# ru-wang/slam-plus-plus

Hardware: AMD Instinct MI355X
Metric: Λ-solve block-nnz/sec + batch GN iters/sec, Venice BA, 1→8 MI355X (higher is better)
Workload: dtype f64; 1 GPU; venice871-shaped synthetic BA (871 cams, 530304 points, 2838740 observations, LM-damped); nnzb=3369915, n=1596138, mode=schur+dense, n_reduced=5226, schur_pairs=12875640, parallelism=single GPU

## Files before the change

slam_plus_plus_amd/csrc/spp_api.cpp:

```cpp

#include "spp_internal.h"
#include <string.h>
#include <new>

using namespace spp;

namespace spp {

void phases_reset(spp_ctx *ctx)
{
	if(!(ctx->flags & SPP_FLAG_PROFILE))
		return;
	if(!ctx->timer.created) {
		for(int i = 0; i < 2 * SPP_N_PHASES; ++ i)
			SPP_HIP_CHECK(hipEventCreate(&ctx->timer.ev[i]));
		ctx->timer.created = true;
	}
	for(int i = 0; i < SPP_N_PHASES; ++ i) {
		ctx->timer.used[i] = false;
		ctx->phase_ms[i] = 0;
	}
	ctx->dom_used = 0;
	ctx->dom_flops = 0;
}
// ... 23 lines not shown
			continue;
		float ms = 0;
		if(hipEventElapsedTime(&ms, ctx->timer.ev[2 * i], ctx->timer.ev[2 * i + 1]) == hipSuccess)
			ctx->phase_ms[i] = ms;
	}
}

void dom_begin(spp_ctx *ctx)
{
	if(!(ctx->flags & SPP_FLAG_PROFILE))
		return;
	if(ctx->dom_used + 2 > ctx->dom_events.size()) {
		size_t old = ctx->dom_events.size();
		ctx->dom_events.resize(old + 64);
		for(size_t i = old; i < ctx->dom_events.size(); ++ i)
			SPP_HIP_CHECK(hipEventCreate(&ctx->dom_events[i]));
	}
	SPP_HIP_CHECK(hipEventRecord(ctx->dom_events[ctx->dom_used], ctx->stream));
}

void dom_end(spp_ctx *ctx, double flops)
{
	if(!(ctx->flags & SPP_FLAG_PROFILE))
		return;
	SPP_HIP_CHECK(hipEventRecord(ctx->dom_events[ctx->dom_used + 1], ctx->stream));
	ctx->dom_used += 2;
	ctx->dom_flops += flops;
}

}

#define SPP_TRY(ctx) try {
#define SPP_CATCH(ctx) } catch(const spp::Error &e) { if(ctx) (ctx)->last_error = e.what(); return e.code; } \
	catch(const std::bad_alloc &) { if(ctx) (ctx)->last_error = "host allocation failed"; return SPP_E_NOMEM; } \
	catch(const std::exception &e) { if(ctx) (ctx)->last_error = e.what(); return SPP_E_HIP; }

extern "C" {

const char *spp_version(void)
{
	return "slam_plus_plus_amd 0.1 (gfx950, fp64)";
}

spp_ctx *spp_create(int device, int flags)
{
	int count = 0;
	if(hipGetDeviceCount(&count) != hipSuccess || count <= 0 || device < 0 || device >= count)
		return nullptr;
	if(hipSetDevice(device) != hipSuccess)
		return nullptr;
	spp_ctx *ctx = new(std::nothrow) spp_ctx;
	if(!ctx)
		return nullptr;
	ctx->device = device;
	ctx->flags = flags;
	if(hipStreamCreateWithFlags(&ctx->stream, hipStreamNonBlocking) != hipSuccess) {
		delete ctx;
		return nullptr;
	}
	ctx->own_stream = true;
	return ctx;
}

int spp_free_memory(spp_ctx *ctx)
{
	if(!ctx)
		return SPP_E_BADARG;
	SPP_TRY(ctx)
	(void)hipSetDevice(ctx->device);
	(void)hipStreamSynchronize(ctx->stream);
	ctx->schur.release_all();
	sparse_release(ctx);
	assemble_release(ctx);
	ctx->dense.tinv.release();
	ctx->dense.tinv_all.release();
	ctx->dense.xtmp.release();
	ctx->dense.la_cnt.release();
	ctx->dense.la_trace.release();
	ctx->geom_partial.release();
	ctx->dense.flags.release();
	ctx->dense.trsv_pay.release();
	ctx->dense.trsv_m.release();
	ctx->dense.tail_pub.release();
	ctx->dense.tail_order.release();
	ctx->dense.tail_order_tr = ctx->dense.tail_order_tc = 0;
	ctx->dense.tail_dinv.release();
	ctx->dense.tail_epoch = 0;
	ctx->dense.epoch = 0;
	ctx->dense.sync.release();
	ctx->dense.fuse_cnt.release();
	ctx->dense.fuse_expect.clear();
	ctx->dense.sync_epoch = 0;
	ctx->d_vals.release();
	ctx->d_rhs.release();
	ctx->mode = -1;
	return SPP_OK;
	SPP_CATCH(ctx)
}

void spp_destroy(spp_ctx *ctx)
{
	if(!ctx)
		return;
	if(ctx->plan_trash.joinable())
		ctx->plan_trash.join();
	spp_free_memory(ctx);
	ctx->dense.info.release();
	if(ctx->dense.aux) {
		dense_aux_park(ctx->device, ctx->dense.aux);
		(void)hipEventDestroy(ctx->dense.ev[0]);
		(void)hipEventDestroy(ctx->dense.ev[1]);
	}
	if(ctx->dense.chain) {
		(void)hipStreamDestroy(ctx->dense.chain);
		if(ctx->dense.ev_chain)
			(void)hipEventDestroy(ctx->dense.ev_chain);
	}
	if(ctx->dense.h_chain_err)
		(void)hipHostFree(ctx->dense.h_chain_err);
	if(ctx->h_staging)
		(void)hipHostFree(ctx->h_staging);
	if(ctx->timer.created)
		for(int i = 0; i < 2 * SPP_N_PHASES; ++ i)
			(void)hipEventDestroy(ctx->timer.ev[i]);
	for(size_t i = 0; i < ctx->dom_events.size(); ++ i)
		(void)hipEventDestroy(ctx->dom_events[i]);
	if(ctx->own_stream && ctx->stream)
		(void)hipStreamDestroy(ctx->stream);
	delete ctx;
}

int spp_last_error(const spp_ctx *ctx, char *buf, size_t buf_size)
{
	if(!ctx || !buf || !buf_size)
		return SPP_E_BADARG;
	strncpy(buf, ctx->last_error.c_str(), buf_size - 1);
	buf[buf_size - 1] = 0;
	return SPP_OK;
}

double *spp_host_staging(spp_ctx *ctx, int64_t n_doubles)
{
	if(!ctx || n_doubles < 0)
		return nullptr;
	if((size_t)n_doubles <= ctx->h_staging_cap && ctx->h_staging)
		return ctx->h_staging;
	(void)hipSetDevice(ctx->device);
	(void)hipStreamSynchronize(ctx->stream);
	if(ctx->h_staging) {
		(void)hipHostFree(ctx->h_staging);
		ctx->h_staging = nullptr;
		ctx->h_staging_cap = 0;
	}
	const size_t want = (size_t)(n_doubles > 0 ? n_doubles : 1);
	if(hipHostMalloc((void**)&ctx->h_staging, want * sizeof(double), hipHostMallocDefault) != hipSuccess) {
		(void)hipGetLastError();
		ctx->h_staging = nullptr;
		ctx->last_error = "hipHostMalloc of the staging buffer failed";
		return nullptr;
	}
	ctx->h_staging_cap = want;
	return ctx->h_staging;
}

int spp_set_stream(spp_ctx *ctx, void *hip_stream)
{
// ... 774 lines not shown
```

slam_plus_plus_amd/csrc/spp_dense.hip:

```cpp

#include "spp_internal.h"
#include "spp_tiles.h"
#include "spp_dense_dev.h"
#include <stdio.h>
#include <stdlib.h>
#include <string.h>
#include <algorithm>
#include <vector>
#include <mutex>

namespace spp {


constexpr int BK = 16;
constexpr int LDS_STRIDE = 18;

template <int BM, int BN, int WM, int WN, int MODE, int DEPTH, int BKT, int SC1 = 0>
__device__ __forceinline__ void gemm_tn_tile(const int64_t m0, const int64_t n0, int64_t M, int64_t N, int K,
	const double *__restrict__ A, int64_t lda, const double *B, int64_t ldb, double *C, int64_t ldc, double *gemm_lds)
{
	constexpr int NWM = BM / WM, NWN = BN / WN, NT = NWM * NWN * 64;
	constexpr int TA = WM / 16, TB = WN / 16;
	constexpr int PPC = BKT / 2, LSTR = BKT + 2;
	constexpr int PA = (BM * PPC) / NT, PB = (BN * PPC) / NT;
// ... 1176 lines not shown
	SPP_HIP_CHECK(hipEventRecord(dw.ev[1], sb));
	SPP_HIP_CHECK(hipEventRecord(dw.ev_chain, sc));
	SPP_HIP_CHECK(hipStreamWaitEvent(s, dw.ev[1], 0));
	SPP_HIP_CHECK(hipStreamWaitEvent(s, dw.ev_chain, 0));
	SPP_HIP_CHECK(hipGetLastError());
	if(tracing) {
		std::vector<long long> h((size_t)12 * nsteps + 16);
		SPP_HIP_CHECK(hipMemcpyAsync(h.data(), dw.la_trace.p, h.size() * sizeof(long long), hipMemcpyDeviceToHost, s));
		SPP_HIP_CHECK(hipStreamSynchronize(s));
		fprintf(stderr, "[spp] lookahead factorization, %d steps: potrf start / duration / gap to the next start (us)\n", a.nsteps);
		for(int k = 0; k < a.nsteps; ++ k)
			fprintf(stderr, "  k %2d  start %8.1f  potrf %5.1f  publish %4.1f | b1 seen +%4.1f  done +%4.1f | c1 seen +%4.1f  done +%4.1f | step %5.1f\n", k,
				(h[8 * k] - h[0]) * 0.01, (h[8 * k + 2] - h[8 * k]) * 0.01, (h[8 * k + 1] - h[8 * k + 2]) * 0.01,
				(h[8 * k + 3] - h[8 * k + 1]) * 0.01, (h[8 * k + 4] - h[8 * k + 1]) * 0.01, (h[8 * k + 5] - h[8 * k + 1]) * 0.01,
				(h[8 * k + 6] - h[8 * k + 1]) * 0.01, k + 1 < a.nsteps ? (h[8 * (k + 1)] - h[8 * k]) * 0.01 : 0.0);
		fprintf(stderr, "[spp] per step: panel (rest) done / bulk launch: first tile starts, priority tiles done, last tile done, busy workgroup-us (all relative to potrf(0) start)\n");
		for(int k = 0; k < a.nsteps; ++ k) {
			const long long *b = h.data() + 8 * nsteps + 8 + 4 * k;
			fprintf(stderr, "  k %2d  panel done %8.1f | bulk start %8.1f  pri done %8.1f  end %8.1f  busy %9.1f\n", k, h[8 * k + 7] ? (h[8 * k + 7] - h[0]) * 0.01 : 0.0,
				b[1] ? (b[0] - h[0]) * 0.01 : 0.0, b[3] ? (b[3] - h[0]) * 0.01 : 0.0, b[1] ? (b[1] - h[0]) * 0.01 : 0.0, b[2] * 0.01);
		}
	}
}

void dense_factor_steps(spp_ctx *ctx, double *d_A, int64_t ld, int64_t n, int64_t rows, int64_t ncols,
	int64_t nsteps, bool has_rhs)
{
	ensure_dense_work(ctx, nsteps);
	ctx->dense.tail_rows_last = 0;
	hipStreamCaptureStatus cs = hipStreamCaptureStatusNone;
	const bool capturing = hipStreamIsCapturing(ctx->stream, &cs) != hipSuccess || cs != hipStreamCaptureStatusNone;
	if(!capturing && la_usable(ctx, nsteps)) {
		dense_factor_lookahead(ctx, d_A, ld, n, rows, ncols, nsteps, has_rhs);
		ctx->dense.tinv_half = 0;
		return;
	}
	ctx->dense.tinv_half = nsteps;
	const bool flags = !capturing && nsteps >= 4 && flag_schedule_usable(ctx);
	dense_factor_steps_enqueue(ctx, d_A, ld, n, rows, ncols, nsteps, has_rhs, flags, !capturing);
}

static void flag_signal(hipStream_t st, int *flag, int value)
{
	hipLaunchKernelGGL(flag_signal_kernel, dim3(1), dim3(64), 0, st, flag, value);
}

static FlagWait make_flag_wait(spp_ctx *ctx, const int *flag, int value, double timeout_ms = 500.0)
{
	return FlagWait{flag, value, ctx->dense.info.p + 2, (long long)(timeout_ms * 1e5)};
}

static void flag_wait(spp_ctx *ctx, hipStream_t st, const int *flag, int value, double timeout_ms)
{
	hipLaunchKernelGGL(flag_wait_kernel, dim3(1), dim3(64), 0, st, make_flag_wait(ctx, flag, value, timeout_ms));
}

static bool flag_schedule_selftest(spp_ctx *ctx)
{
	DenseWork &dw = ctx->dense;
	hipStream_t st[2] = {ctx->stream, dw.aux};
	dw.sync.reserve(16);
	SPP_HIP_CHECK(hipMemsetAsync(dw.sync.p, 0, 16 * sizeof(int), ctx->stream));
	SPP_HIP_CHECK(hipStreamSynchronize(ctx->stream));
	for(int p = 0; p < 2; ++ p) {
		flag_wait(ctx, st[p], dw.sync.p + p, 1, 20.0);
		flag_signal(st[1 - p], dw.sync.p + p, 1);
	}
	for(int i = 0; i < 2; ++ i)
		SPP_HIP_CHECK(hipStreamSynchronize(st[i]));
	int h_abort = 0;
	SPP_HIP_CHECK(hipMemcpy(&h_abort, dw.info.p + 2, sizeof(int), hipMemcpyDeviceToHost));
	if(h_abort) {
		SPP_HIP_CHECK(hipMemset(dw.info.p + 2, 0, sizeof(int)));
		return false;
	}
	return true;
}

static bool flag_schedule_usable(spp_ctx *ctx)
{
	static int sched = -1;
	if(sched < 0) {
		const char *e = getenv("SPP_DENSE_SCHED");
		sched = e ? atoi(e) : 1;
	}
	if(!sched)
		return false;
	DenseWork &dw = ctx->dense;
	if(dw.sync_state == 0 || dw.sync_stream != ctx->stream) {
		hipStreamCaptureStatus cs = hipStreamCaptureStatusNone;
		if(hipStreamIsCapturing(ctx->stream, &cs) != hipSuccess || cs != hipStreamCaptureStatusNone)
			return false;
		dw.sync_state = flag_schedule_selftest(ctx) ? 1 : -1;
		dw.sync_stream = ctx->stream;
	}
	return dw.sync_state == 1;
}

static int dense_tail_rows()
{
	static int v = -1;
	if(v < 0) {
		const char *e = getenv("SPP_TAIL_ROWS"), *on = getenv("SPP_DENSE_TAIL");
		v = (on && !atoi(on)) ? 0 : (e ? atoi(e) : 44);
	}
	return v;
}

static bool dense_tail_applies(spp_ctx *ctx, int64_t rows, int64_t nsteps)
{
	return !ctx->dense.tail_disabled && nsteps * NB >= rows && !(ctx->dense.ident_from >= 0 && ctx->dense.ident_from < rows);
}

static bool launch_dense_tail(spp_ctx *ctx, double *d_A, int64_t ld, int64_t rows, int64_t ncols, int64_t nsteps, int64_t k, bool has_rhs)
{
	static int enabled = -1;
	if(enabled < 0) {
		const char *e = getenv("SPP_DENSE_TAIL");
		enabled = e ? atoi(e) : 1;
	}
	DenseWork &dw = ctx->dense;
	const int64_t c1 = (k + 1) * NB;
	if(!enabled || dw.tail_disabled || k + 1 >= nsteps || nsteps * NB < rows || (dw.ident_from >= 0 && dw.ident_from < rows))
		return false;
	const int Tr = (int)(nsteps - (k + 1)), Tc = (int)((ncols - c1 + NB - 1) / NB);
	if(Tr < 1 || Tc < Tr || Tc > Tr + 1)
		return false;
	const int ntile = Tr * Tc - Tr * (Tr - 1) / 2;
	static int max_rows = -1;
	if(max_rows < 0) {
		const char *e = getenv("SPP_TAIL_ROWS");
		max_rows = e ? atoi(e) : 44;
	}
	if(Tr > max_rows)
		return false;
	hipStream_t s = ctx->stream;
	static uint64_t attr_seen = 0;
	if(first_on_this_device(attr_seen))
		SPP_HIP_CHECK(hipFuncSetAttribute((const void*)dense_tail_kernel, hipFuncAttributeMaxDynamicSharedMemorySize,
			TAIL_LDS_DOUBLES * (int)sizeof(double)));
	if(dw.tail_pub.cap < (size_t)Tr * Tc) {
		dw.tail_pub.reserve(std::max<size_t>((size_t)Tr * Tc, 24 * 25));
		SPP_HIP_CHECK(hipMemsetAsync(dw.tail_pub.p, 0, dw.tail_pub.cap * sizeof(int), s));
		dw.tail_epoch = 0;
	}
	if(dw.tail_dinv.cap < (size_t)Tr * 8 * 256)
		dw.tail_dinv.reserve(std::max<size_t>((size_t)Tr * 8 * 256, (size_t)24 * 8 * 256));
	if(++ dw.tail_epoch >= (1 << 26)) {
		SPP_HIP_CHECK(hipMemsetAsync(dw.tail_pub.p, 0, dw.tail_pub.cap * sizeof(int), s));
		dw.tail_epoch = 1;
	}
	if(dw.tail_order_tr != Tr || dw.tail_order_tc != Tc) {
		static double beta = -1;
		if(beta < 0) {
			const char *e = getenv("SPP_TAIL_ORDER_BETA");
			beta = e ? atof(e) : 0.0;
		}
		std::vector<std::pair<double, int> > key;
		for(int i = 0; i < Tr; ++ i)
			for(int j = i; j < Tc; ++ j)
				key.push_back(std::make_pair((double)i + beta * (double)j, (i << 16) | j));
		std::stable_sort(key.begin(), key.end(), [](const std::pair<double, int> &x, const std::pair<double, int> &y) { return x.first < y.first; });
		std::vector<int> &order = dw.tail_order_host;
		order.resize(key.size());
		for(size_t q = 0; q < key.size(); ++ q)
			order[q] = key[q].second;
		dw.tail_order.upload(order, s);
		dw.tail_order_tr = Tr;
		dw.tail_order_tc = Tc;
	}
	TailArgs a;
	a.order = dw.tail_order.p;
	a.A = d_A;
	a.ld = ld;
	a.rows = rows;
	a.ncols = ncols;
	a.c0 = c1;
	a.have_pre = (k >= 0) ? 1 : 0;
	a.Tr = Tr;
	a.Tc = Tc;
	a.has_rhs = has_rhs ? 1 : 0;
	a.tinv = dw.tinv_all.p + (size_t)(k + 1) * NB * NB;
	a.dbuf = dw.tail_dinv.p;
	a.pub = dw.tail_pub.p;
	a.epoch = dw.tail_epoch;
	a.info = dw.info.p;
	a.abort = dw.info.p + 2;
	static long long tail_timeout = -1;
	if(tail_timeout < 0) {
		const char *e = getenv("SPP_TAIL_TIMEOUT_TICKS");
		tail_timeout = e ? atoll(e) : (long long)(500.0 * 1e5);
	}
	a.timeout_ticks = tail_timeout;
	static int trace_env = -1;
	if(trace_env < 0) {
		const char *e = getenv("SPP_TAIL_TRACE");
		trace_env = e ? atoi(e) : 0;
	}
	static int launches = 0;
	DevBuf<long long> trace;
	a.trace = nullptr;
	if(trace_env && ++ launches == trace_env) {
		trace.reserve((size_t)Tr * 8);
		SPP_HIP_CHECK(hipMemsetAsync(trace.p, 0, (size_t)Tr * 8 * sizeof(long long), s));
		a.trace = trace.p;
	}
	dom_begin(ctx);
	hipLaunchKernelGGL(dense_tail_kernel, dim3((unsigned)ntile), dim3(POTRF_THREADS), TAIL_LDS_DOUBLES * sizeof(double), s, a);
	{
		const double m = (double)(rows - c1);
		dom_end(ctx, m * m * m / 3.0 + (a.have_pre ? (double)NB * m * (m + 1.0) : 0.0) + 2.0 * m * m);
	}
	dw.tail_rows_last = Tr;
	SPP_HIP_CHECK(hipGetLastError());
	if(a.trace) {
		std::vector<long long> h((size_t)Tr * 8);
		SPP_HIP_CHECK(hipStreamSynchronize(s));
		SPP_HIP_CHECK(hipMemcpy(h.data(), trace.p, h.size() * sizeof(long long), hipMemcpyDeviceToHost));
		fprintf(stderr, "[spp] streamed tail, %d tile rows (us from the launch's first stamp): diagonal tile: updates complete / factored+inverted | first panel tile: first row tile seen / last seen / last published\n", Tr);
		const long long t0 = h[0];
		for(int i = 0; i < Tr; ++ i)
			fprintf(stderr, "  row %2d  start %7.1f  updated %7.1f  done %7.1f | %7.1f %7.1f %7.1f\n", i, (h[8 * i] - t0) * 0.01, (h[8 * i + 1] - t0) * 0.01,
				(h[8 * i + 2] - t0) * 0.01, h[8 * i + 3] ? (h[8 * i + 3] - t0) * 0.01 : 0.0, h[8 * i + 4] ? (h[8 * i + 4] - t0) * 0.01 : 0.0, h[8 * i + 5] ? (h[8 * i + 5] - t0) * 0.01 : 0.0);
	}
	return true;
}

static void dense_factor_steps_enqueue(spp_ctx *ctx, double *d_A, int64_t ld, int64_t n, int64_t rows, int64_t ncols,
	int64_t nsteps, bool has_rhs, bool use_flags, bool allow_fused)
{
	hipStream_t s = ctx->stream, s2 = ctx->dense.aux;
	hipEvent_t evA = ctx->dense.ev[0], evB = ctx->dense.ev[1];
	DenseWork &dw = ctx->dense;
	const int64_t n_id = (dw.ident_from >= 0 && dw.ident_from < n) ? dw.ident_from : n;
	int ep = 0;
	int64_t step_a = -1, step_b = -1;
	int64_t need_wait_b = -1;
	if(use_flags) {
		if(dw.sync.cap < (size_t)(2 * nsteps + 16)) {
			dw.sync.reserve((size_t)(2 * nsteps + 16));
			SPP_HIP_CHECK(hipMemsetAsync(dw.sync.p, 0, dw.sync.cap * sizeof(int), s));
			dw.sync_epoch = 1;
		}
		ep = ++ dw.sync_epoch;
		SPP_HIP_CHECK(hipEventRecord(evA, s));
		SPP_HIP_CHECK(hipStreamWaitEvent(s2, evA, 0));
	}
	int64_t pend_sig = -1;
	auto record_a = [&](int64_t k) {
		step_a = k;
		if(use_flags)
			pend_sig = k;
		else
			SPP_HIP_CHECK(hipEventRecord(evA, s));
	};
	int64_t pend_sig_b = -1;
	auto wait_a_on_bulk = [&]() {
		if(use_flags && pend_sig_b >= 0) {
			hipLaunchKernelGGL(flag_signal_wait_kernel, dim3(1), dim3(64), 0, s2, dw.sync.p + 2 * pend_sig_b + 1, ep,
				make_flag_wait(ctx, dw.sync.p + 2 * step_a, ep));
			pend_sig_b = -1;
		} else if(use_flags)
			flag_wait(ctx, s2, dw.sync.p + 2 * step_a, ep);
		else
			SPP_HIP_CHECK(hipStreamWaitEvent(s2, evA, 0));
	};
	auto flush_sig_b = [&]() {
		if(pend_sig_b >= 0)
			flag_signal(s2, dw.sync.p + 2 * pend_sig_b + 1, ep);
		pend_sig_b = -1;
	};
	auto record_b = [&](int64_t k) {
		step_b = k;
		if(use_flags)
			pend_sig_b = k;
		else
			SPP_HIP_CHECK(hipEventRecord(evB, s2));
	};
	auto wait_b_now = [&]() {
		if(use_flags && pend_sig_b == step_b)
			flush_sig_b();
		if(use_flags && pend_sig >= 0) {
			flag_signal(s, dw.sync.p + 2 * pend_sig, ep);
			pend_sig = -1;
		}
		if(use_flags)
			flag_wait(ctx, s, dw.sync.p + 2 * step_b + 1, ep);
		else
			SPP_HIP_CHECK(hipStreamWaitEvent(s, evB, 0));
	};
	auto wait_b_deferred = [&]() {
// ... 516 lines not shown
```

slam_plus_plus_amd/csrc/spp_dense_tail.h:

```cpp
#pragma once
#include "spp_dense_dev.h"

namespace spp {

struct TailArgs {
	double *A;
	int64_t ld;
	int64_t rows;
	int64_t ncols;
	int64_t c0;
	int have_pre;
	int Tr, Tc;
	int has_rhs;
	double *tinv;
	double *dbuf;
	int *pub;
	int epoch;
	int *info, *abort;
	long long timeout_ticks;
	long long *trace;
	const int *order;
};

constexpr int TAIL_ABORT_TIMEOUT = 2;

constexpr int TAIL_LDS_DOUBLES = POTRF_LDS_DOUBLES_INV2 + 16;

#ifndef SPP_TAIL_PLAIN_LD
#define SPP_TAIL_PLAIN_LD 0
#endif
__device__ __forceinline__ double tail_ld(const double *p)
{
#if SPP_TAIL_PLAIN_LD
	return __hip_atomic_load(p, __ATOMIC_RELAXED, __HIP_MEMORY_SCOPE_WORKGROUP);
#else
	return __hip_atomic_load(p, __ATOMIC_RELAXED, __HIP_MEMORY_SCOPE_AGENT);
#endif
}

__device__ __noinline__ void tail_first_tile(double *sm, const v4f64 t00, const int lane, int *info, const int64_t k0)
{
	const int l15 = lane & 15, l4 = lane >> 4;
#pragma unroll
	for(int r = 0; r < 4; ++ r)
		sm[(l4 + 4 * r) + l15 * TS] = t00[r];
	if(lane == 0)
		potrf_lds2_fail(sm)[0] = 0;
	__builtin_amdgcn_fence(__ATOMIC_ACQ_REL, "wavefront");
	__builtin_amdgcn_wave_barrier();
	diag_tile_factor<TS>(sm, potrf_lds2_dv(sm), potrf_lds2_gd0(sm), potrf_lds2_dinv(sm), 0, lane, potrf_lds2_fail(sm), info, k0);
}

__global__ __launch_bounds__(POTRF_THREADS)
void dense_tail_kernel(const TailArgs a)
{
	extern __shared__ double sm[];
	const int tid = threadIdx.x, lane = tid & 63, wave = __builtin_amdgcn_readfirstlane(tid >> 6);
	const int l15 = lane & 15, l4 = lane >> 4;
	int *st = (int*)(sm + POTRF_LDS_DOUBLES_INV2);
	const int ord = a.order[blockIdx.x];
	const int ti = ord >> 16, tj = ord & 0xffff;
	const bool diag = ti == tj;
	const int64_t i0 = a.c0 + (int64_t)NB * ti, j0 = a.c0 + (int64_t)NB * tj;
	const int tag = a.epoch << 4;
	auto stamp = [&](int slot) { if(a.trace && tid == 0) a.trace[ti * 8 + slot] = wall_clock64(); };
	if(diag) stamp(0);
	auto pub_count = [&](const int v, const int w) -> int {
		const int cv = ((v >> 4) == a.epoch) ? (v & 15) : 0, cw = ((w >> 4) == a.epoch) ? (w & 15) : 0;
		return cv < cw ? cv : cw;
	};
	auto wait_pub = [&](const int *p, const int *q, const int need) -> int {
		if(tid == 0) {
			const long long t0 = wall_clock64();
			int got = -1;
			for(;;) {
				const int v = __hip_atomic_load(p, __ATOMIC_RELAXED, __HIP_MEMORY_SCOPE_AGENT);
				const int w = q ? __hip_atomic_load(q, __ATOMIC_RELAXED, __HIP_MEMORY_SCOPE_AGENT) : v;
				const int cv = ((v >> 4) == a.epoch) ? (v & 15) : 0, cw = ((w >> 4) == a.epoch) ? (w & 15) : 0;
				const int c = cv < cw ? cv : cw;
				if(c >= need) {
					got = c;
					break;
				}
				if(__hip_atomic_load(a.abort, __ATOMIC_RELAXED, __HIP_MEMORY_SCOPE_AGENT))
					break;
				if(wall_clock64() - t0 > a.timeout_ticks) {
					__hip_atomic_store(a.abort, TAIL_ABORT_TIMEOUT, __ATOMIC_RELAXED, __HIP_MEMORY_SCOPE_AGENT);
					break;
				}
				__builtin_amdgcn_s_sleep(1);
			}
			st[1] = got;
		}
		lds_barrier();
		const int got = st[1];
		lds_barrier();
		return got;
	};
	int ra[4], cb[4];
#pragma unroll
	for(int u = 0; u < 4; ++ u) {
		if(!diag) {
			ra[u] = wave & 7;
			cb[u] = 4 * (wave >> 3) + u;
		} else {
			int q = (wave == 0) ? (u == 0 ? 0 : 36) : wave + 15 * u, c = 0;
			if(q >= 36)
				ra[u] = cb[u] = -1;
			else {
				while(q > c) {
					q -= c + 1;
					++ c;
				}
				ra[u] = q;
				cb[u] = c;
			}
		}
	}
	v4f64 acc[4];
	{
		double *img = sm;
#pragma unroll 4
		for(int q = 0; q < NB * NB / POTRF_THREADS; ++ q) {
			const int e = tid + q * POTRF_THREADS, r = e & (NB - 1), c = e >> 7;
			const int64_t row = i0 + r, col = j0 + c;
			img[r + c * TS] = (col < a.ncols) ? a.A[row + col * a.ld] : ((diag && row == col) ? 1.0 : 0.0);
		}
		lds_barrier();
#pragma unroll
		for(int u = 0; u < 4; ++ u)
#pragma unroll
			for(int r = 0; r < 4; ++ r)
				acc[u][r] = (ra[u] < 0) ? 0.0 : img[(16 * ra[u] + l4 + 4 * r) + (16 * cb[u] + l15) * TS];
		lds_barrier();
	}
	bool pre_first = false;
	{
		const int ek = tid & 15, ec = tid >> 4;
		constexpr int PS = 18;
		const int ekp = 4 * (ek & 3) + (ek >> 2);
		const int kfirst = a.have_pre ? -1 : 0, nst = 8 * (ti - kfirst);
		double va[2], vb[2];
		auto fetch = [&](const int sidx) {
			const int k = kfirst + (sidx >> 3), J = sidx & 7;
			const double *rowp = a.A + (a.c0 + (int64_t)NB * k) + 16 * J + ek;
#pragma unroll
			for(int h = 0; h < 2; ++ h) {
				const int64_t ca = i0 + ec + 64 * h, cb = j0 + ec + 64 * h;
				va[h] = (ca < (diag ? a.ncols : a.rows)) ? tail_ld(rowp + ca * a.ld) : 0.0;
				vb[h] = (!diag && cb < a.ncols) ? tail_ld(rowp + cb * a.ld) : 0.0;
			}
		};
		int avail = a.have_pre ? 8 : 0;
		pre_first = diag && nst > 0 && (nst & 1) == 0 && a.rows - i0 >= 16;
		bool inflight = false;
		for(int sidx = 0; sidx < nst; ++ sidx) {
			const int k = kfirst + (sidx >> 3), J = sidx & 7;
			if(J == 0 && k >= 0)
				avail = 0;
			if(!inflight) {
				if(J >= avail) {
					avail = wait_pub(a.pub + k * a.Tc + ti, a.pub + k * a.Tc + tj, J + 1);
					if(avail < 0)
						return;
				}
				fetch(sidx);
			}
			int pk = -1;
			if(tid == 0 && k >= 0 && J + 1 < 8 && J + 1 >= avail)
				pk = pub_count(__hip_atomic_load(a.pub + k * a.Tc + ti, __ATOMIC_RELAXED, __HIP_MEMORY_SCOPE_AGENT),
					__hip_atomic_load(a.pub + k * a.Tc + tj, __ATOMIC_RELAXED, __HIP_MEMORY_SCOPE_AGENT));
			double *sa = sm + (sidx & 1) * 2 * NB * PS, *sb = diag ? sa : sa + NB * PS;
#pragma unroll
			for(int h = 0; h < 2; ++ h) {
				sa[ekp + (ec + 64 * h) * PS] = va[h];
				if(!diag)
					sb[ekp + (ec + 64 * h) * PS] = vb[h];
			}
			if(tid == 0)
				st[2 + (sidx & 1)] = pk;
			lds_barrier();
			{
				const int seen = st[2 + (sidx & 1)];
				if(seen > avail)
					avail = seen;
			}
			inflight = (sidx + 1 < nst) && (J + 1 < 8) && (J + 1 < avail);
			if(inflight)
				fetch(sidx + 1);
			double fa[4];
#pragma unroll
			for(int u = 0; u < 4; ++ u) {
				if(ra[u] < 0)
					continue;
				double fb[4];
				if(u == 0 || diag) {
					const bool row_live = i0 + 16 * ra[u] + l15 < a.rows;
					const double2 a01 = *(const double2*)(sa + 4 * l4 + (16 * ra[u] + l15) * PS), a23 = *(const double2*)(sa + 4 * l4 + 2 + (16 * ra[u] + l15) * PS);
					fa[0] = row_live ? -a01.x : 0.0;
					fa[1] = row_live ? -a01.y : 0.0;
					fa[2] = row_live ? -a23.x : 0.0;
					fa[3] = row_live ? -a23.y : 0.0;
				}
				{
					const double2 b01 = *(const double2*)(sb + 4 * l4 + (16 * cb[u] + l15) * PS), b23 = *(const double2*)(sb + 4 * l4 + 2 + (16 * cb[u] + l15) * PS);
					fb[0] = b01.x;
					fb[1] = b01.y;
					fb[2] = b23.x;
					fb[3] = b23.y;
				}
#pragma unroll
				for(int kk = 0; kk < 4; ++ kk)
					acc[u] = __builtin_amdgcn_mfma_f64_16x16x4f64(fa[kk], fb[kk], acc[u], 0, 0, 0);
				if(u == 0 && pre_first && sidx == nst - 1 && wave == 0) {
					tail_first_tile(sm, acc[0], lane, a.info, i0);
				}
			}
		}
		lds_barrier();
	}
	if(diag) stamp(1);
	double *T = sm;
#pragma unroll
	for(int u = 0; u < 4; ++ u)
#pragma unroll
		for(int r = 0; r < 4; ++ r)
			if(ra[u] >= 0 && !(pre_first && wave == 0 && u == 0))
				T[(16 * ra[u] + l4 + 4 * r) + (16 * cb[u] + l15) * TS] = acc[u][r];
	lds_barrier();
	if(diag) {
		const int64_t nv = a.rows - i0;
		const int n_valid = (int)(nv < 0 ? 0 : (nv > NB ? NB : nv));
		PotrfPub pb;
		pb.flag = a.pub + ti * a.Tc + ti;
		pb.base = tag;
		pb.dbuf = a.dbuf + (size_t)ti * 8 * 256;
		pb.abort = a.abort;
		potrf_diag_body<false, 1, 2, true>(a.A + i0 + i0 * a.ld, a.ld, n_valid, (a.has_rhs && n_valid < NB) ? 1 : 0,
			a.tinv + (size_t)ti * NB * NB, a.info, i0, sm, pb, pre_first ? 1 : 0);
		stamp(2);
		return;
	}
	double *Dv = T + NB * TS;
	double *Rr = Dv + 16 * PT;
	const double *Rii = a.A + i0 + i0 * a.ld;
	int avail = 0;
	bool inflight = false;
	double dvr = 0, rr[2] = {0, 0};
	auto fetch_panel = [&](const int J) {
		if(tid < 256)
			dvr = tail_ld(a.dbuf + ((size_t)ti * 8 + J) * 256 + tid);
#pragma unroll
		for(int h = 0; h < 2; ++ h) {
			const int e = tid + POTRF_THREADS * h, k = e & 15, c = e >> 4;
			if(e < 16 * (NB - 16 * (J + 1)))
				rr[h] = tail_ld(Rii + (16 * J + k) + (int64_t)(16 * (J + 1) + c) * a.ld);
		}
	};
	for(int J = 0; J < 8; ++ J) {
		if(!inflight) {
			if(J >= avail) {
				avail = wait_pub(a.pub + ti * a.Tc + ti, nullptr, J + 1);
				if(avail < 0)
					return;
			}
			fetch_panel(J);
		}
		if(tj == ti + 1 && J == 0) stamp(3);
		if(tj == ti + 1 && J == 7) stamp(4);
		int pk = -1;
		if(tid == 0 && J + 1 < 8 && J + 1 >= avail) {
			const int v = __hip_atomic_load(a.pub + ti * a.Tc + ti, __ATOMIC_RELAXED, __HIP_MEMORY_SCOPE_AGENT);
			pk = pub_count(v, v);
		}
		if(tid < 256)
			Dv[(tid & 15) + (tid >> 4) * PT] = dvr;
#pragma unroll
		for(int h = 0; h < 2; ++ h) {
			const int e = tid + POTRF_THREADS * h;
			if(e < 16 * (NB - 16 * (J + 1)))
				Rr[(e & 15) + (e >> 4) * PT] = rr[h];
		}
		if(tid == 0)
			st[2 + (J & 1)] = pk;
		lds_barrier();
		{
			const int seen = st[2 + (J & 1)];
			if(seen > avail)
				avail = seen;
		}
		inflight = (J + 1 < 8) && (J + 1 < avail);
		if(inflight)
			fetch_panel(J + 1);
		if(wave < 8) {
			double *Y = T + 16 * J + (16 * wave) * TS;
			const v4f64 x = tile_atb(Dv, 1, PT, Y, 1, TS, lane);
			__builtin_amdgcn_fence(__ATOMIC_ACQ_REL, "wavefront");
			__builtin_amdgcn_wave_barrier();
			const int64_t col = j0 + 16 * wave + l15;
#pragma unroll
			for(int r = 0; r < 4; ++ r) {
				Y[(l4 + 4 * r) + l15 * TS] = x[r];
				if(col < a.ncols)
					__hip_atomic_store(&a.A[(i0 + 16 * J + l4 + 4 * r) + col * a.ld], x[r], __ATOMIC_RELAXED, __HIP_MEMORY_SCOPE_AGENT);
			}
		}
		lds_barrier();
		{
			const int b = wave & 7;
			double xb[4];
#pragma unroll
			for(int kk = 0; kk < 4; ++ kk)
				xb[kk] = T[16 * J + (4 * kk + l4) + (16 * b + l15) * TS];
			auto row_update = [&](const int I) {
				const double *Ra = Rr + 16 * (I - J - 1) * PT;
				v4f64 d = (v4f64){0, 0, 0, 0};
#pragma unroll
				for(int kk = 0; kk < 4; ++ kk)
					d = __builtin_amdgcn_mfma_f64_16x16x4f64(Ra[(4 * kk + l4) + l15 * PT], xb[kk], d, 0, 0, 0);
				double *D = T + 16 * I + (16 * b) * TS;
#pragma unroll
				for(int r = 0; r < 4; ++ r)
					D[(l4 + 4 * r) + l15 * TS] -= d[r];
			};
			{
				const int I = J + 1 + (wave >> 3);
				if(I < 8)
					row_update(I);
			}
			if(wave < 8)
				asm volatile("s_waitcnt vmcnt(0)" ::: "memory");
			lds_barrier();
			if(tid == 0)
				__hip_atomic_store(a.pub + ti * a.Tc + tj, tag | (J + 1), __ATOMIC_RELAXED, __HIP_MEMORY_SCOPE_AGENT);
			for(int I = J + 3 + (wave >> 3); I < 8; I += 2)
				row_update(I);
			lds_barrier();
		}
		if(tj == ti + 1 && J == 7) stamp(5);
	}
}

}
```

slam_plus_plus_amd/csrc/spp_internal.h:

```cpp
#pragma once

#include <hip/hip_runtime.h>
#include <stdint.h>
#include <string>
#include <vector>
#include <sys/mman.h>
#include <utility>
#include <new>
#include <exception>
#include <thread>
#include <stdexcept>
#include <algorithm>
#include <string.h>
#include <chrono>
#include <stdio.h>
#include <stdlib.h>
#include "../../include/spp_hip.h"

namespace spp {

struct Error : std::runtime_error {
	int code;
	Error(int c, const std::string &what) : std::runtime_error(what), code(c) {}
};
// ... 138 lines not shown
			*items[i].powned = false;
		}
	}
};

struct Structure {
	int64_t nb = 0, n = 0, nnzb = 0, nvals = 0;
	HVec<int64_t> col_ptr, row_idx, blk_off, base;
	HVec<int32_t> dim;
};

struct SaccItem {
	int32_t beg, end;
	int32_t kind;
	int32_t pad;
	int64_t dst;
	int64_t aoff;
};

struct SchurPlan {
	int dp = 0, dl = 0;
	int64_t nc = 0, nl = 0;
	int64_t nl_total = 0;
	int64_t no = 0;
	int64_t n_red = 0, ld = 0;
	int64_t n_sblk = 0;
	int64_t n_pairs = 0;
	int64_t n_items = 0, n_multi = 0;
	bool add_A = true;
	bool u_landmark_major = true;
	bool factored = true;
	bool sparse_S = false;
	bool mis = false;
	Structure s_st;
	DevBuf<int64_t> sblk_voff;
	std::vector<int64_t> pose_block;
	std::vector<int64_t> lm_block;
	std::vector<uint8_t> is_lm;
	DevBuf<int32_t> lm_ptr;
	DevBuf<int32_t> bs_ptr;
	int64_t n_bs = 0;
	DevBuf<int64_t> lm_coff;
	DevBuf<int64_t> lm_rbase;
	DevBuf<int32_t> obs_pose;
	DevBuf<int32_t> obs_lm;
	DevBuf<int64_t> obs_off;
	DevBuf<int64_t> pose_rbase;
	DevBuf<int32_t> cam_ptr;
	DevBuf<int32_t> cam_obs;
	DevBuf<int32_t> obs_wpos;
	DevBuf<SaccItem> items;
	DevBuf<int32_t> xcd_beg;
	int32_t xcd_max_items = 0;
	DevBuf<int32_t> sblk_i1, sblk_i2;
	DevBuf<int64_t> sblk_aoff;
	DevBuf<int32_t> pair_a, pair_b;
	DevBuf<int32_t> multi_blk;
	DevBuf<int32_t> multi_ptr;
	DevBuf<double> cinv;
	DevBuf<double> lfac;
	DevBuf<double> W;
	DevBuf<double> Up;
	DevBuf<double> xw;
	DevBuf<double> partial;
	DevBuf<double> S;
	void release_all();
};

struct DenseWork {
	DevBuf<double> tinv;
	DevBuf<int> info;
	DevBuf<double> tinv_all;
	int64_t tinv_half = 0;
	DevBuf<double> xtmp;
	DevBuf<int> flags;
	DevBuf<int> tail_pub;
	DevBuf<double> tail_dinv;
	int tail_epoch = 0;
	DevBuf<int> tail_order;
	std::vector<int> tail_order_host;
	int tail_order_tr = 0, tail_order_tc = 0;
	int tail_rows_last = 0;
	bool tail_disabled = false;
	DevBuf<double> trsv_m;
	DevBuf<double> trsv_pay;
	uint64_t epoch = 0;
	int *h_chain_err = nullptr;
	hipStream_t aux = nullptr;
	hipEvent_t ev[2] = {nullptr, nullptr};
	DevBuf<int> sync;
	DevBuf<int> fuse_cnt;
	std::vector<int> fuse_expect;
	bool fuse_dirty = false;
	int64_t ident_from = -1;
	hipStream_t chain = nullptr;
	hipEvent_t ev_chain = nullptr;
	DevBuf<int> la_cnt;
	DevBuf<long long> la_trace;
	int la_state = 0;
	int la_reserve = 0;
	int la_ncu = 0;
	int sync_epoch = 0;
	int sync_state = 0;
	hipStream_t sync_stream = nullptr;
};

struct SparsePlan;

struct AssemblePlan;

struct PhaseTimer {
	hipEvent_t ev[2 * SPP_N_PHASES];
	bool used[SPP_N_PHASES];
	bool created = false;
};

}

struct spp_ctx {
	int device = 0;
	int flags = 0;
	hipStream_t stream = nullptr;
	bool own_stream = false;
	std::string last_error;
	int mode = -1;
	int shard_rank = 0, shard_world = 1;
	spp::Structure st;
	std::vector<int64_t> order;
	std::thread plan_trash;
	spp::SchurPlan schur;
	spp::DenseWork dense;
	spp::SparsePlan *sparse = nullptr;
	spp::AssemblePlan *assemble = nullptr;
	spp::DevBuf<double> d_vals, d_rhs;
	double *h_staging = nullptr;
	size_t h_staging_cap = 0;
	spp::DevBuf<double> geom_partial;
	spp::PhaseTimer timer;
	double phase_ms[SPP_N_PHASES] = {0};
	std::vector<hipEvent_t> dom_events;
	size_t dom_used = 0;
	double dom_flops = 0;
	int64_t factor_flops = 0, solve_bytes = 0, factor_nnz = 0;
};

namespace spp {

void se2_linearize(spp_ctx *ctx, int64_t ne, const int32_t *d_v0, const int32_t *d_v1, const double *d_poses,
	const double *d_meas, double *d_J0, double *d_J1, double *d_r);
double se2_update(spp_ctx *ctx, int64_t nv, double *d_poses, const double *d_dx, bool apply);
double edge_chi2(spp_ctx *ctx, int64_t ne, int rd, const double *d_r, const double *d_Om);
void edge_robust_weights(spp_ctx *ctx, int64_t ne, int rd, int kind, double scale, double param, const double *d_r, double *d_w);
double edge_hessian_maxdiag(spp_ctx *ctx, int64_t ne, int rd, int d0, int d1, const double *d_J0, const double *d_J1,
	const double *d_Om);
double lm_gain_denominator(spp_ctx *ctx, int64_t n, const double *d_dx, const double *d_rhs, double alpha);
void se3_linearize(spp_ctx *ctx, int64_t ne, const int32_t *d_v0, const int32_t *d_v1, const double *d_poses,
	const double *d_meas, double *d_J0, double *d_J1, double *d_r);
double se3_update(spp_ctx *ctx, int64_t nv, double *d_poses, const double *d_dx, bool apply);
void ba_linearize(spp_ctx *ctx, int64_t no, const int32_t *d_cam_of, const int32_t *d_pt_of, const double *d_cams,
	const double *d_intr, const double *d_pts, const double *d_meas, double *d_J0, double *d_J1, double *d_r);
double ba_update(spp_ctx *ctx, int64_t nc, double *d_cams, const int64_t *d_cam_dxoff, int64_t np, double *d_pts,
	const int64_t *d_pt_dxoff, const double *d_dx, int64_t n_dx, bool apply);

void min_degree_order(int64_t nb, const int64_t *col_ptr, const int64_t *row_idx, std::vector<int64_t> &order);
void nested_dissection_order(int64_t nb, const int64_t *col_ptr, const int64_t *row_idx, std::vector<int64_t> &order);
void build_schur_plan(spp_ctx *ctx, bool sparse_S, bool mis = false);
// ... 103 lines not shown
```

Baseline: 1.124 billion block-nnz/s.

## Add persistent task-queue kernel for dense tail with split tile segments

Adds a persistent dense-tail kernel sized to the compute-unit count. Each block pulls tasks from an atomic ticket counter, and tile updates can be split into segments that park partial results in global memory for a later task to resume. A host-built task table orders and checks these dependencies. The aim is better load balance and less idle time on the triangular tail factorisation than one block per tile, at the cost of extra global round-trips and spin-waits. The task kernel is off by default (SPP_TAIL_SCHED=0), but this change also switches the flag-based dense schedule (SPP_DENSE_SCHED) off by default, which changes the path that runs.

Measured after the change: 1.125 billion block-nnz/s (median of 4 runs). Within noise of the previous version (+0.1%).

```diff
diff --git a/slam_plus_plus_amd/csrc/spp_api.cpp b/slam_plus_plus_amd/csrc/spp_api.cpp
--- a/slam_plus_plus_amd/csrc/spp_api.cpp
+++ b/slam_plus_plus_amd/csrc/spp_api.cpp
@@ -129,6 +129,8 @@
 	ctx->dense.trsv_pay.release();
 	ctx->dense.trsv_m.release();
 	ctx->dense.tail_pub.release();
+	ctx->dense.tail_park.release();
+	ctx->dense.tail_ticket.release();
 	ctx->dense.tail_order.release();
 	ctx->dense.tail_order_tr = ctx->dense.tail_order_tc = 0;
 	ctx->dense.tail_dinv.release();
diff --git a/slam_plus_plus_amd/csrc/spp_dense.hip b/slam_plus_plus_amd/csrc/spp_dense.hip
--- a/slam_plus_plus_amd/csrc/spp_dense.hip
+++ b/slam_plus_plus_amd/csrc/spp_dense.hip
@@ -1282,7 +1282,7 @@
 	static int sched = -1;
 	if(sched < 0) {
 		const char *e = getenv("SPP_DENSE_SCHED");
-		sched = e ? atoi(e) : 1;
+		sched = e ? atoi(e) : 0;
 	}
 	if(!sched)
 		return false;
@@ -1310,6 +1310,47 @@
 static bool dense_tail_applies(spp_ctx *ctx, int64_t rows, int64_t nsteps)
 {
 	return !ctx->dense.tail_disabled && nsteps * NB >= rows && !(ctx->dense.ident_from >= 0 && ctx->dense.ident_from < rows);
+}
+
+static void tail_task_table(std::vector<int> &order, int Tr, int Tc, int pre, int seg, double split)
+{
+	if(Tc + pre > 63)
+		throw Error(SPP_E_UNSUPPORTED, "streamed dense factor: more tile columns than the task table holds (SPP_TAIL_ROWS)");
+	struct Seg { double key; int code; };
+	std::vector<Seg> t;
+	for(int i = 0; i < Tr; ++ i)
+		for(int j = i; j < Tc; ++ j) {
+			const int ns = i + pre;
+			int s0 = 0;
+			for(int c = 1; c < ns; ++ c) {
+				const bool cut = (seg == 2) || (seg == 1 && c == (int)(split * i) + pre);
+				if(!cut)
+					continue;
+				t.push_back(Seg{(double)(c - pre) + 0.5, (i << 24) | (j << 16) | (s0 << 8) | c});
+				s0 = c;
+			}
+			t.push_back(Seg{(double)i, (i << 24) | (j << 16) | (s0 << 8) | ns});
+		}
+	std::stable_sort(t.begin(), t.end(), [](const Seg &x, const Seg &y) { return x.key < y.key; });
+	order.resize(t.size());
+	std::vector<int> own((size_t)Tr * Tc, -1), parked((size_t)Tr * Tc * 64, -1);
+	for(size_t q = 0; q < t.size(); ++ q) {
+		const int c = order[q] = t[q].code, i = c >> 24, j = (c >> 16) & 0xff, s1 = c & 0xff;
+		(s1 == i + pre ? own[(size_t)i * Tc + j] : parked[((size_t)i * Tc + j) * 64 + s1]) = (int)q;
+	}
+	for(size_t q = 0; q < t.size(); ++ q) {
+		const int c = order[q], i = c >> 24, j = (c >> 16) & 0xff, s0 = (c >> 8) & 0xff, s1 = c & 0xff;
+		bool ok = s0 < s1 || (s0 == 0 && s1 == 0);
+		for(int k = std::max(s0 - pre, 0); k < s1 - pre; ++ k)
+			ok = ok && own[(size_t)k * Tc + i] >= 0 && own[(size_t)k * Tc + i] < (int)q && own[(size_t)k * Tc + j] >= 0 && own[(size_t)k * Tc + j] < (int)q;
+		if(s0 > 0)
+			ok = ok && parked[((size_t)i * Tc + j) * 64 + s0] >= 0 && parked[((size_t)i * Tc + j) * 64 + s0] < (int)q;
+		if(s1 == i + pre && j > i)
+			ok = ok && own[(size_t)i * Tc + i] < (int)q;
+		if(!ok)
+			throw Error(SPP_E_STATE, "streamed dense factor: the task table breaks its order (segment of tile (" +
+				std::to_string(i) + ", " + std::to_string(j) + "), steps " + std::to_string(s0) + " .. " + std::to_string(s1) + ")");
+	}
 }
 
 static bool launch_dense_tail(spp_ctx *ctx, double *d_A, int64_t ld, int64_t rows, int64_t ncols, int64_t nsteps, int64_t k, bool has_rhs)
@@ -1336,41 +1377,67 @@
 		return false;
 	hipStream_t s = ctx->stream;
 	static uint64_t attr_seen = 0;
-	if(first_on_this_device(attr_seen))
+	if(first_on_this_device(attr_seen)) {
 		SPP_HIP_CHECK(hipFuncSetAttribute((const void*)dense_tail_kernel, hipFuncAttributeMaxDynamicSharedMemorySize,
 			TAIL_LDS_DOUBLES * (int)sizeof(double)));
+		SPP_HIP_CHECK(hipFuncSetAttribute((const void*)dense_tail_tasks_kernel, hipFuncAttributeMaxDynamicSharedMemorySize,
+			TAIL_LDS_DOUBLES * (int)sizeof(double)));
+	}
 	if(dw.tail_pub.cap < (size_t)Tr * Tc) {
 		dw.tail_pub.reserve(std::max<size_t>((size_t)Tr * Tc, 24 * 25));
+		dw.tail_park.reserve(dw.tail_pub.cap);
 		SPP_HIP_CHECK(hipMemsetAsync(dw.tail_pub.p, 0, dw.tail_pub.cap * sizeof(int), s));
+		SPP_HIP_CHECK(hipMemsetAsync(dw.tail_park.p, 0, dw.tail_park.cap * sizeof(int), s));
 		dw.tail_epoch = 0;
+	}
+	if(!dw.tail_ticket.p) {
+		dw.tail_ticket.reserve(4);
+		SPP_HIP_CHECK(hipMemsetAsync(dw.tail_ticket.p, 0, 4 * sizeof(int), s));
 	}
 	if(dw.tail_dinv.cap < (size_t)Tr * 8 * 256)
 		dw.tail_dinv.reserve(std::max<size_t>((size_t)Tr * 8 * 256, (size_t)24 * 8 * 256));
-	if(++ dw.tail_epoch >= (1 << 26)) {
+	if(++ dw.tail_epoch >= (1 << 24)) {
 		SPP_HIP_CHECK(hipMemsetAsync(dw.tail_pub.p, 0, dw.tail_pub.cap * sizeof(int), s));
+		SPP_HIP_CHECK(hipMemsetAsync(dw.tail_park.p, 0, dw.tail_park.cap * sizeof(int), s));
 		dw.tail_epoch = 1;
 	}
+	static int sched = -1, seg = -1;
+	static double split = -1;
+	if(sched < 0) {
+		const char *e = getenv("SPP_TAIL_SCHED");
+		sched = e ? atoi(e) : 0;
+		e = getenv("SPP_TAIL_SEG");
+		seg = e ? atoi(e) : 1;
+		e = getenv("SPP_TAIL_SPLIT");
+		split = e ? atof(e) : 0.5;
+	}
 	if(dw.tail_order_tr != Tr || dw.tail_order_tc != Tc) {
-		static double beta = -1;
-		if(beta < 0) {
-			const char *e = getenv("SPP_TAIL_ORDER_BETA");
-			beta = e ? atof(e) : 0.0;
-		}
-		std::vector<std::pair<double, int> > key;
-		for(int i = 0; i < Tr; ++ i)
-			for(int j = i; j < Tc; ++ j)
-				key.push_back(std::make_pair((double)i + beta * (double)j, (i << 16) | j));
-		std::stable_sort(key.begin(), key.end(), [](const std::pair<double, int> &x, const std::pair<double, int> &y) { return x.first < y.first; });
 		std::vector<int> &order = dw.tail_order_host;
-		order.resize(key.size());
-		for(size_t q = 0; q < key.size(); ++ q)
-			order[q] = key[q].second;
+		if(!sched) {
+			static double beta = -1;
+			if(beta < 0) {
+				const char *e = getenv("SPP_TAIL_ORDER_BETA");
+				beta = e ? atof(e) : 0.0;
+			}
+			std::vector<std::pair<double, int> > key;
+			for(int i = 0; i < Tr; ++ i)
+				for(int j = i; j < Tc; ++ j)
+					key.push_back(std::make_pair((double)i + beta * (double)j, (i << 16) | j));
+			std::stable_sort(key.begin(), key.end(), [](const std::pair<double, int> &x, const std::pair<double, int> &y) { return x.first < y.first; });
+			order.resize(key.size());
+			for(size_t q = 0; q < key.size(); ++ q)
+				order[q] = key[q].second;
+		} else
+			tail_task_table(order, Tr, Tc, k >= 0 ? 1 : 0, seg, split);
 		dw.tail_order.upload(order, s);
 		dw.tail_order_tr = Tr;
 		dw.tail_order_tc = Tc;
 	}
 	TailArgs a;
 	a.order = dw.tail_order.p;
+	a.park = dw.tail_park.p;
+	a.ticket = dw.tail_ticket.p;
+	a.ntask = (int)dw.tail_order_host.size();
 	a.A = d_A;
 	a.ld = ld;
 	a.rows = rows;
@@ -1406,7 +1473,13 @@
 		a.trace = trace.p;
 	}
 	dom_begin(ctx);
-	hipLaunchKernelGGL(dense_tail_kernel, dim3((unsigned)ntile), dim3(POTRF_THREADS), TAIL_LDS_DOUBLES * sizeof(double), s, a);
+	if(sched) {
+		if(!dw.tail_ncu)
+			SPP_HIP_CHECK(hipDeviceGetAttribute(&dw.tail_ncu, hipDeviceAttributeMultiprocessorCount, ctx->device));
+		hipLaunchKernelGGL(dense_tail_tasks_kernel, dim3((unsigned)std::min(a.ntask, dw.tail_ncu)), dim3(POTRF_THREADS),
+			TAIL_LDS_DOUBLES * sizeof(double), s, a);
+	} else
+		hipLaunchKernelGGL(dense_tail_kernel, dim3((unsigned)ntile), dim3(POTRF_THREADS), TAIL_LDS_DOUBLES * sizeof(double), s, a);
 	{
 		const double m = (double)(rows - c1);
 		dom_end(ctx, m * m * m / 3.0 + (a.have_pre ? (double)NB * m * (m + 1.0) : 0.0) + 2.0 * m * m);
diff --git a/slam_plus_plus_amd/csrc/spp_dense_tail.h b/slam_plus_plus_amd/csrc/spp_dense_tail.h
--- a/slam_plus_plus_amd/csrc/spp_dense_tail.h
+++ b/slam_plus_plus_amd/csrc/spp_dense_tail.h
@@ -20,6 +20,9 @@
 	long long timeout_ticks;
 	long long *trace;
 	const int *order;
+	int *park;
+	int *ticket;
+	int ntask;
 };
 
 constexpr int TAIL_ABORT_TIMEOUT = 2;
@@ -51,32 +54,32 @@
 	diag_tile_factor<TS>(sm, potrf_lds2_dv(sm), potrf_lds2_gd0(sm), potrf_lds2_dinv(sm), 0, lane, potrf_lds2_fail(sm), info, k0);
 }
 
-__global__ __launch_bounds__(POTRF_THREADS)
-void dense_tail_kernel(const TailArgs a)
+template <bool TASKS>
+__device__ __forceinline__ bool tail_tile(const TailArgs a, const int ti, const int tj, const int s0, const int s1)
 {
 	extern __shared__ double sm[];
 	const int tid = threadIdx.x, lane = tid & 63, wave = __builtin_amdgcn_readfirstlane(tid >> 6);
 	const int l15 = lane & 15, l4 = lane >> 4;
 	int *st = (int*)(sm + POTRF_LDS_DOUBLES_INV2);
-	const int ord = a.order[blockIdx.x];
-	const int ti = ord >> 16, tj = ord & 0xffff;
+	const int ns = ti + a.have_pre, sb = TASKS ? s0 : 0, se = TASKS ? s1 : ns;
+	const bool own = !TASKS || se == ns, resume = TASKS && sb > 0;
 	const bool diag = ti == tj;
 	const int64_t i0 = a.c0 + (int64_t)NB * ti, j0 = a.c0 + (int64_t)NB * tj;
 	const int tag = a.epoch << 4;
 	auto stamp = [&](int slot) { if(a.trace && tid == 0) a.trace[ti * 8 + slot] = wall_clock64(); };
-	if(diag) stamp(0);
+	if(diag && sb == 0) stamp(0);
 	auto pub_count = [&](const int v, const int w) -> int {
 		const int cv = ((v >> 4) == a.epoch) ? (v & 15) : 0, cw = ((w >> 4) == a.epoch) ? (w & 15) : 0;
 		return cv < cw ? cv : cw;
 	};
-	auto wait_pub = [&](const int *p, const int *q, const int need) -> int {
+	auto wait_pub = [&](const int *p, const int *q, const int need, const int sh = 4) -> int {
 		if(tid == 0) {
 			const long long t0 = wall_clock64();
 			int got = -1;
 			for(;;) {
 				const int v = __hip_atomic_load(p, __ATOMIC_RELAXED, __HIP_MEMORY_SCOPE_AGENT);
 				const int w = q ? __hip_atomic_load(q, __ATOMIC_RELAXED, __HIP_MEMORY_SCOPE_AGENT) : v;
-				const int cv = ((v >> 4) == a.epoch) ? (v & 15) : 0, cw = ((w >> 4) == a.epoch) ? (w & 15) : 0;
+				const int cv = ((v >> sh) == a.epoch) ? (v & ((1 << sh) - 1)) : 0, cw = ((w >> sh) == a.epoch) ? (w & ((1 << sh) - 1)) : 0;
 				const int c = cv < cw ? cv : cw;
 				if(c >= need) {
 					got = c;
@@ -119,12 +122,14 @@
 	}
 	v4f64 acc[4];
 	{
+		if(resume && wait_pub(a.park + ti * a.Tc + tj, nullptr, sb, 6) < 0)
+			return false;
 		double *img = sm;
 #pragma unroll 4
 		for(int q = 0; q < NB * NB / POTRF_THREADS; ++ q) {
 			const int e = tid + q * POTRF_THREADS, r = e & (NB - 1), c = e >> 7;
 			const int64_t row = i0 + r, col = j0 + c;
-			img[r + c * TS] = (col < a.ncols) ? a.A[row + col * a.ld] : ((diag && row == col) ? 1.0 : 0.0);
+			img[r + c * TS] = (col < a.ncols) ? (resume ? tail_ld(a.A + row + col * a.ld) : a.A[row + col * a.ld]) : ((diag && row == col) ? 1.0 : 0.0);
 		}
 		lds_barrier();
 #pragma unroll
@@ -152,9 +157,10 @@
 			}
 		};
 		int avail = a.have_pre ? 8 : 0;
-		pre_first = diag && nst > 0 && (nst & 1) == 0 && a.rows - i0 >= 16;
+		const int send = 8 * se;
+		pre_first = diag && own && se > sb && (nst & 1) == 0 && a.rows - i0 >= 16;
 		bool inflight = false;
-		for(int sidx = 0; sidx < nst; ++ sidx) {
+		for(int sidx = 8 * sb; sidx < send; ++ sidx) {
 			const int k = kfirst + (sidx >> 3), J = sidx & 7;
 			if(J == 0 && k >= 0)
 				avail = 0;
@@ -162,7 +168,7 @@
 				if(J >= avail) {
 					avail = wait_pub(a.pub + k * a.Tc + ti, a.pub + k * a.Tc + tj, J + 1);
 					if(avail < 0)
-						return;
+						return false;
 				}
 				fetch(sidx);
 			}
@@ -185,7 +191,7 @@
 				if(seen > avail)
 					avail = seen;
 			}
-			inflight = (sidx + 1 < nst) && (J + 1 < 8) && (J + 1 < avail);
+			inflight = (sidx + 1 < send) && (J + 1 < 8) && (J + 1 < avail);
 			if(inflight)
 				fetch(sidx + 1);
 			double fa[4];
@@ -212,12 +218,34 @@
 #pragma unroll
 				for(int kk = 0; kk < 4; ++ kk)
 					acc[u] = __builtin_amdgcn_mfma_f64_16x16x4f64(fa[kk], fb[kk], acc[u], 0, 0, 0);
-				if(u == 0 && pre_first && sidx == nst - 1 && wave == 0) {
-					tail_first_tile(sm, acc[0], lane, a.info, i0);
-				}
-			}
-		}
-		lds_barrier();
+			}
+		}
+		if(pre_first && wave == 0) {
+			tail_first_tile(sm, acc[0], lane, a.info, i0);
+		}
+		lds_barrier();
+	}
+	if(TASKS && !own) {
+		double *img = sm;
+#pragma unroll
+		for(int u = 0; u < 4; ++ u)
+#pragma unroll
+			for(int r = 0; r < 4; ++ r)
+				if(ra[u] >= 0)
+					img[(16 * ra[u] + l4 + 4 * r) + (16 * cb[u] + l15) * TS] = acc[u][r];
+		lds_barrier();
+#pragma unroll 4
+		for(int q = 0; q < NB * NB / POTRF_THREADS; ++ q) {
+			const int e = tid + q * POTRF_THREADS, r = e & (NB - 1), c = e >> 7;
+			const int64_t col = j0 + c;
+			if(col < a.ncols && (!diag || (r >> 4) <= (c >> 4)))
+				__hip_atomic_store(&a.A[(i0 + r) + col * a.ld], img[r + c * TS], __ATOMIC_RELAXED, __HIP_MEMORY_SCOPE_AGENT);
+		}
+		asm volatile("s_waitcnt vmcnt(0)" ::: "memory");
+		lds_barrier();
+		if(tid == 0)
+			__hip_atomic_store(a.park + ti * a.Tc + tj, (a.epoch << 6) | se, __ATOMIC_RELAXED, __HIP_MEMORY_SCOPE_AGENT);
+		return true;
 	}
 	if(diag) stamp(1);
 	double *T = sm;
@@ -239,7 +267,7 @@
 		potrf_diag_body<false, 1, 2, true>(a.A + i0 + i0 * a.ld, a.ld, n_valid, (a.has_rhs && n_valid < NB) ? 1 : 0,
 			a.tinv + (size_t)ti * NB * NB, a.info, i0, sm, pb, pre_first ? 1 : 0);
 		stamp(2);
-		return;
+		return true;
 	}
 	double *Dv = T + NB * TS;
 	double *Rr = Dv + 16 * PT;
@@ -262,7 +290,7 @@
 			if(J >= avail) {
 				avail = wait_pub(a.pub + ti * a.Tc + ti, nullptr, J + 1);
 				if(avail < 0)
-					return;
+					return false;
 			}
 			fetch_panel(J);
 		}
@@ -339,6 +367,51 @@
 		}
 		if(tj == ti + 1 && J == 7) stamp(5);
 	}
-}
-
-}
+	return true;
+}
+
+__global__ __launch_bounds__(POTRF_THREADS)
+void dense_tail_kernel(const TailArgs a)
+{
+	const int ord = a.order[blockIdx.x];
+	const int ti = ord >> 16, tj = ord & 0xffff;
+	tail_tile<false>(a, ti, tj, 0, ti + a.have_pre);
+}
+
+__device__ __noinline__ bool tail_task(const TailArgs &a, int task)
+{
+	task = __builtin_amdgcn_readfirstlane(task);
+	return tail_tile<true>(a, task >> 24, (task >> 16) & 0xff, (task >> 8) & 0xff, task & 0xff);
+}
+
+__global__ __launch_bounds__(POTRF_THREADS)
+void dense_tail_tasks_kernel(const TailArgs a)
+{
+	extern __shared__ double sm[];
+	int *st = (int*)(sm + POTRF_LDS_DOUBLES_INV2);
+	const int tid = threadIdx.x;
+	for(;;) {
+		if(tid == 0) {
+			int t = -1;
+			if(!__hip_atomic_load(a.abort, __ATOMIC_RELAXED, __HIP_MEMORY_SCOPE_AGENT)) {
+				t = __hip_atomic_fetch_add(a.ticket, 1, __ATOMIC_RELAXED, __HIP_MEMORY_SCOPE_AGENT);
+				if(t >= a.ntask)
+					t = -1;
+			}
+			st[4] = t;
+		}
+		lds_barrier();
+		const int t = __builtin_amdgcn_readfirstlane(st[4]);
+		lds_barrier();
+		if(t < 0)
+			break;
+		if(!tail_task(a, a.order[t]))
+			break;
+	}
+	if(tid == 0 && __hip_atomic_fetch_add(a.ticket + 1, 1, __ATOMIC_RELAXED, __HIP_MEMORY_SCOPE_AGENT) == (int)gridDim.x - 1) {
+		__hip_atomic_store(a.ticket, 0, __ATOMIC_RELAXED, __HIP_MEMORY_SCOPE_AGENT);
+		__hip_atomic_store(a.ticket + 1, 0, __ATOMIC_RELAXED, __HIP_MEMORY_SCOPE_AGENT);
+	}
+}
+
+}
diff --git a/slam_plus_plus_amd/csrc/spp_internal.h b/slam_plus_plus_amd/csrc/spp_internal.h
--- a/slam_plus_plus_amd/csrc/spp_internal.h
+++ b/slam_plus_plus_amd/csrc/spp_internal.h
@@ -244,6 +244,9 @@
 	int tail_order_tr = 0, tail_order_tc = 0;
 	int tail_rows_last = 0;
 	bool tail_disabled = false;
+	DevBuf<int> tail_park;
+	DevBuf<int> tail_ticket;
+	int tail_ncu = 0;
 	DevBuf<double> trsv_m;
 	DevBuf<double> trsv_pay;
 	uint64_t epoch = 0;
```
